# PlanNoa/video_super_resolution

Hardware: NVIDIA B200
Metric: sr_frames_per_s_4x_1080p_out (higher is better)
Workload: dtype bf16

## Files before the change

video_super_resolution_b200/csrc/fused_down.cuh:

```cuda
#pragma once
#include "igemm.cuh"

namespace vsr {

constexpr int kFusedEpiWarps = 16;
constexpr int kFusedWdWarp = 2 + kFusedEpiWarps;
constexpr int kFusedBWarp = kFusedWdWarp + 1;
constexpr int kFusedThreads = 32 * (kFusedBWarp + 1);
constexpr int kFusedMaxStages = 16;
constexpr int kWdGroupBytes = 128 * 128 * 2;
constexpr int kWdRingBytes = 2 * kWdGroupBytes;
constexpr int kWtChunkBytes = 32 * 32 * 2;
constexpr int kHBytes = 128 * 128 * 2;
constexpr int kXchgBytes = 3 * 4 * 16 * 8 * 4;

struct alignas(64) FusedDownParams {
  CUtensorMap hr_maps[kMaxSources];
  CUtensorMap h0_map;
  CUtensorMap wt_map;
  CUtensorMap wd_map;
  int32_t nsrc;
  int32_t num_stages;
  int32_t tiles_x, tiles_y, batch;
  int32_t lr_h, lr_w;
  const float* tran_bias;
  const float* down_bias;
  float* part;
  void* lr_out;
};

__device__ __forceinline__ void tmem_ld8(uint32_t taddr, uint32_t (&v)[8]) {
  asm volatile("tcgen05.ld.sync.aligned.32x32b.x8.b32 {%0, %1, %2, %3, %4, %5, %6, %7}, [%8];"
               : "=r"(v[0]), "=r"(v[1]), "=r"(v[2]), "=r"(v[3]), "=r"(v[4]), "=r"(v[5]), "=r"(v[6]), "=r"(v[7])
               : "r"(taddr)
               : "memory");
}

template <bool HAS_TRAN>
inline size_t fused_down_smem_bytes(int nsrc, int num_stages) {
  size_t wt = HAS_TRAN ? ((size_t)nsrc * kWtChunkBytes + 1023) / 1024 * 1024 : 0;
  size_t stage = HAS_TRAN ? 16384 : 2 * 16384;
  return 1024 + kWdRingBytes + wt + (HAS_TRAN ? kHBytes : 0) + (size_t)num_stages * stage + 1024 + kXchgBytes;
}

template <bool HAS_TRAN>
__global__ void __launch_bounds__(kFusedThreads, 1)
fused_down_kernel(const __grid_constant__ FusedDownParams p) {
  constexpr int kStageBytes = HAS_TRAN ? 16384 : 2 * 16384;
  constexpr int kTmemCols = HAS_TRAN ? 512 : 256;
  constexpr uint32_t kDB = HAS_TRAN ? 256 : 0;

  extern __shared__ uint8_t smem_raw[];
  uint8_t* smem = smem_raw + ((1024u - (smem_u32(smem_raw) & 1023u)) & 1023u);
  uint8_t* s_wd = smem;
  uint8_t* s_wt = s_wd + kWdRingBytes;
  const int wt_region = HAS_TRAN ? ((p.nsrc * kWtChunkBytes + 1023) / 1024 * 1024) : 0;
  uint8_t* s_h = s_wt + wt_region;
  uint8_t* s_a = s_h + (HAS_TRAN ? kHBytes : 0);
  uint8_t* tail = s_a + p.num_stages * kStageBytes;
  uint64_t* full_bar = reinterpret_cast<uint64_t*>(tail);
  uint64_t* empty_bar = full_bar + kFusedMaxStages;
  uint64_t* w_full = empty_bar + kFusedMaxStages;
  uint64_t* wd_full = w_full + 1;
  uint64_t* wd_empty = wd_full + 2;
  uint64_t* da_full = wd_empty + 2;
  uint64_t* da_empty = da_full + 2;
  uint64_t* h_full = da_empty + 2;
  uint64_t* h_empty = h_full + 1;
  uint64_t* db_full = h_empty + 1;
  uint64_t* db_empty = db_full + 2;
  uint32_t* tmem_ptr = reinterpret_cast<uint32_t*>(db_empty + 2);
  float* s_bias = reinterpret_cast<float*>(tail + 512);
  float* s_down = s_bias + 36;
  float4* s_x = reinterpret_cast<float4*>(tail + 1024);

  const int cta = blockIdx.x, ncta = gridDim.x;
  const int warp = threadIdx.x >> 5;
  const int lane = threadIdx.x & 31;
  const int total_tiles = p.tiles_x * p.tiles_y * p.batch;

  if (threadIdx.x == 0) {
    for (int s = 0; s < p.num_stages; ++s) {
      mbar_init(&full_bar[s], 1);
      mbar_init(&empty_bar[s], 1);
    }
    mbar_init(w_full, 1);
    for (int s = 0; s < 2; ++s) {
      mbar_init(&wd_full[s], 1);
      mbar_init(&wd_empty[s], 1);
      mbar_init(&da_full[s], 1);
      mbar_init(&da_empty[s], kFusedEpiWarps);
      mbar_init(&db_full[s], 1);
      mbar_init(&db_empty[s], kFusedEpiWarps);
    }
    mbar_init(h_full, kFusedEpiWarps);
    mbar_init(h_empty, 1);
    fence_barrier_init();
  }
  if (warp == 1) tmem_alloc<kTmemCols>(tmem_ptr);
  if (HAS_TRAN)
    for (int i = threadIdx.x; i < 33; i += kFusedThreads) s_bias[i] = p.tran_bias[i];
  for (int i = threadIdx.x; i < 33; i += kFusedThreads) s_down[i] = p.down_bias[i];
  tc_fence_before();
  __syncthreads();
  tc_fence_after();
  const uint32_t tmem_base = *tmem_ptr;

  auto tile_coord = [&](int tile, int& x0, int& y0, int& b) {
    x0 = (tile % p.tiles_x) * 16;
    int r = tile / p.tiles_x;
    y0 = (r % p.tiles_y) * 8;
    b = r / p.tiles_y;
  };

  if (warp == 0) {
    {
      if (HAS_TRAN && elect_one()) {
        mbar_expect_tx(w_full, (uint32_t)(p.nsrc * kWtChunkBytes));
        for (int j = 0; j < p.nsrc; ++j) tma_load_2d(s_wt + j * kWtChunkBytes, &p.wt_map, w_full, j * 32, 0);
      }
      __syncwarp();
      int s = 0;
      uint32_t phase = 0;
      for (int tile = cta; tile < total_tiles; tile += ncta) {
        int x0, y0, b;
        tile_coord(tile, x0, y0, b);
        for (int half = 0; half < 2; ++half) {
          if (HAS_TRAN) {
            for (int sp = half * 8; sp < half * 8 + 8; sp += 2) {
              for (int j = 0; j < p.nsrc; ++j) {
                mbar_wait(&empty_bar[s], phase ^ 1);
                if (elect_one()) {
                  mbar_expect_tx(&full_bar[s], kStageBytes);
                  tma_load_4d(s_a + s * kStageBytes, &p.hr_maps[j], &full_bar[s], 0, x0, y0, b * 8 + (sp >> 1));
                }
                __syncwarp();
                if (++s == p.num_stages) { s = 0; phase ^= 1; }
              }
            }
          } else {
            for (int g = half * 2; g < half * 2 + 2; ++g) {
              mbar_wait(&empty_bar[s], phase ^ 1);
              if (elect_one()) {
                mbar_expect_tx(&full_bar[s], kStageBytes);
                tma_load_4d(s_a + s * kStageBytes, &p.h0_map, &full_bar[s], 0, x0, y0, b * 8 + 2 * g);
                tma_load_4d(s_a + s * kStageBytes + 16384, &p.h0_map, &full_bar[s], 0, x0, y0, b * 8 + 2 * g + 1);
              }
              __syncwarp();
              if (++s == p.num_stages) { s = 0; phase ^= 1; }
            }
          }
        }
      }
    }
  } else if (warp == 1 || (HAS_TRAN && warp == kFusedBWarp)) {
    {
    constexpr uint32_t idesc_a = make_idesc(32);
    constexpr uint32_t idesc_b = make_idesc(128);
    if (HAS_TRAN && warp == 1) mbar_wait(w_full, 0);
    tc_fence_after();
    int s = 0;
    uint32_t phase = 0;
    uint32_t n_a[2] = {0, 0}, n_b[2] = {0, 0}, n_h = 0, n_wd = 0;
    int tb = 0;
    const uint64_t dA = make_smem_desc<128>(smem_u32(s_a));
    const uint64_t dWt = make_smem_desc<64>(smem_u32(s_wt));
    const uint64_t dH = make_smem_desc<128>(smem_u32(s_h));
    const uint64_t dWd = make_smem_desc<128>(smem_u32(s_wd));

    auto issue_a = [&](int g) {
      const int buf = g & 1;
      mbar_wait(&da_empty[buf], (n_a[buf] & 1) ^ 1);
      tc_fence_after();
      for (int pair = 0; pair < 2; ++pair)
        for (int j = 0; j < p.nsrc; ++j) {
          mbar_wait(&full_bar[s], phase);
          tc_fence_after();
          const uint64_t a0 = dA + (uint64_t)((s * kStageBytes) >> 4);
          const uint64_t b0 = dWt + (uint64_t)((j * kWtChunkBytes) >> 4);
          const uint32_t d0 = tmem_base + (uint32_t)(buf * 128 + pair * 64);
          if (elect_one()) {
            const uint32_t acc = (uint32_t)(j != 0);
            umma_bf16(d0, a0, b0, idesc_a, acc);
            umma_bf16(d0, a0 + 2, b0 + 2, idesc_a, 1u);
            umma_bf16(d0 + 32, a0 + 4, b0, idesc_a, acc);
            umma_bf16(d0 + 32, a0 + 6, b0 + 2, idesc_a, 1u);
            umma_commit(&empty_bar[s]);
            if (pair == 1 && j == p.nsrc - 1) umma_commit(&da_full[buf]);
          }
          __syncwarp();
          if (++s == p.num_stages) { s = 0; phase ^= 1; }
        }
      ++n_a[buf];
    };
    auto issue_b = [&](int g) {
      uint64_t a0;
      if (HAS_TRAN) {
        mbar_wait(h_full, n_h & 1);
        a0 = dH;
      } else {
        mbar_wait(&full_bar[s], phase);
        a0 = dA + (uint64_t)((s * kStageBytes) >> 4);
      }
      if (g == 0) mbar_wait(&db_empty[tb], (n_b[tb] & 1) ^ 1);
      const int wslot = (int)(n_wd & 1);
      mbar_wait(&wd_full[wslot], (n_wd >> 1) & 1);
      tc_fence_after();
      const uint32_t d = tmem_base + kDB + (uint32_t)(tb * 128);
      const uint64_t b0 = dWd + (uint64_t)((wslot * kWdGroupBytes) >> 4);
      if (elect_one()) {
#pragma unroll
        for (int kc = 0; kc < 2; ++kc)
#pragma unroll
          for (int k = 0; k < 4; ++k)
            umma_bf16(d, a0 + (uint64_t)(kc * 1024 + k * 2), b0 + (uint64_t)(kc * 1024 + k * 2), idesc_b,
                      (uint32_t)((g | kc | k) != 0));
        umma_commit(&wd_empty[wslot]);
        if (HAS_TRAN) umma_commit(h_empty);
        else umma_commit(&empty_bar[s]);
        if (g == 3) umma_commit(&db_full[tb]);
      }
      __syncwarp();
      ++n_wd;
      if (HAS_TRAN) ++n_h;
      else if (++s == p.num_stages) { s = 0; phase ^= 1; }
      if (g == 3) { ++n_b[tb]; tb ^= 1; }
    };

    for (int tile = cta; tile < total_tiles; tile += ncta) {
      if (HAS_TRAN) {
        if (warp == 1) {
          for (int g = 0; g < 4; ++g) issue_a(g);
        } else {
          for (int g = 0; g < 4; ++g) issue_b(g);
        }
      } else {
        for (int g = 0; g < 4; ++g) issue_b(g);
      }
    }
    }
  } else if (warp == kFusedWdWarp) {
    uint32_t n_wd = 0;
    for (int tile = cta; tile < total_tiles; tile += ncta)
      for (int g = 0; g < 4; ++g) {
        const int slot = n_wd & 1;
        mbar_wait(&wd_empty[slot], ((n_wd >> 1) & 1) ^ 1);
        if (elect_one()) {
          mbar_expect_tx(&wd_full[slot], kWdGroupBytes);
          tma_load_2d(s_wd + slot * kWdGroupBytes, &p.wd_map, &wd_full[slot], (2 * g) * 64, 0);
          tma_load_2d(s_wd + slot * kWdGroupBytes + 16384, &p.wd_map, &wd_full[slot], (2 * g + 1) * 64, 0);
        }
        __syncwarp();
        ++n_wd;
      }
  } else if (warp >= 2 && warp < 2 + kFusedEpiWarps) {
    const int q = warp & 3;
    const int sub = (warp - 2) >> 2;
    const int row = q * 32 + lane;
    const uint32_t lane_base = tmem_base + ((uint32_t)(q * 32) << 16);
    uint32_t m_a[2] = {0, 0}, m_b[2] = {0, 0}, m_h = 0;
    int tb = 0;
    const PreluCfg pc = make_prelu(HAS_TRAN ? s_bias[32] : 1.0f, 1);
    for (int tile = cta; tile < total_tiles; tile += ncta) {
      int x0, y0, b;
      tile_coord(tile, x0, y0, b);
      const int Yb = y0 + (row >> 4), Xb = x0 + (row & 15);
      const bool in_tensor = (Yb <= p.lr_h) && (Xb <= p.lr_w);
      if (HAS_TRAN) {
#pragma unroll 1
        for (int g = 0; g < 4; ++g) {
          const int buf = g & 1;
          mbar_wait_poll(&da_full[buf], m_a[buf] & 1);
          tc_fence_after();
          uint32_t o[16];
          uint32_t v[32];
          tmem_ld32(lane_base + (uint32_t)(buf * 128 + sub * 32), v);
          tmem_ld_wait();
          tc_fence_before();
          mbar_arrive_warp(&da_empty[buf]);
          const int s16 = g * 4 + sub, ry = s16 >> 2, rx = s16 & 3;
          const bool ring = (Yb == 0 && ry < 2) || (Yb == p.lr_h && ry >= 2) || (Xb == 0 && rx < 2) ||
                            (Xb == p.lr_w && rx >= 2);
          convert32(v, s_bias, pc, o);
          if (__builtin_expect(!(in_tensor && !ring), 0)) zero16(o);
          ++m_a[buf];
          mbar_wait(h_empty, (m_h & 1) ^ 1);
          uint8_t* hrow = s_h + (sub >> 1) * 16384 + (row >> 3) * 1024 + (row & 7) * 128;
#pragma unroll
          for (int j = 0; j < 4; ++j) {
            const int piece = (sub & 1) * 4 + j;
            *reinterpret_cast<uint4*>(hrow + ((piece ^ (row & 7)) << 4)) =
                make_uint4(o[4 * j], o[4 * j + 1], o[4 * j + 2], o[4 * j + 3]);
          }
          fence_async_smem();
          mbar_arrive_warp(h_full);
          ++m_h;
        }
      }
      mbar_wait_poll(&db_full[tb], m_b[tb] & 1);
      tc_fence_after();
      uint32_t v[4][8];
#pragma unroll
      for (int t = 0; t < 4; ++t) tmem_ld8(lane_base + kDB + (uint32_t)(tb * 128 + t * 32 + sub * 8), v[t]);
      tmem_ld_wait();
      tc_fence_before();
      mbar_arrive_warp(&db_empty[tb]);
      const int xl = lane & 15, half = lane >> 4;
      float comb[2][8];
#pragma unroll
      for (int dy = 0; dy < 2; ++dy)
#pragma unroll
        for (int k = 0; k < 8; ++k) {
          const float right = __uint_as_float(v[dy * 2 + 1][k]);
          const float from_right = __shfl_down_sync(0xffffffffu, right, 1);
          comb[dy][k] = __uint_as_float(v[dy * 2][k]) + (xl < 15 ? from_right : 0.0f);
        }
      float below[8];
#pragma unroll
      for (int k = 0; k < 8; ++k) below[k] = __shfl_down_sync(0xffffffffu, comb[1][k], 16);
      if (half == 0 && q > 0) {
        float4* x = s_x + (((q - 1) * 4 + sub) * 16 + xl) * 2;
        x[0] = make_float4(comb[1][0], comb[1][1], comb[1][2], comb[1][3]);
        x[1] = make_float4(comb[1][4], comb[1][5], comb[1][6], comb[1][7]);
      }
      asm volatile("bar.sync 1, %0;" ::"n"(32 * kFusedEpiWarps) : "memory");
      if (half == 1 && q < 3) {
        const float4* x = s_x + ((q * 4 + sub) * 16 + xl) * 2;
        const float4 x0v = x[0], x1v = x[1];
        below[0] = x0v.x; below[1] = x0v.y; below[2] = x0v.z; below[3] = x0v.w;
        below[4] = x1v.x; below[5] = x1v.y; below[6] = x1v.z; below[7] = x1v.w;
      }
      asm volatile("bar.sync 1, %0;" ::"n"(32 * kFusedEpiWarps) : "memory");
      const int rr = 2 * q + half;
      if (rr < 7 && xl < 15 && in_tensor && Yb < p.lr_h && Xb < p.lr_w) {
        const float slope = s_down[32];
        float r[8];
#pragma unroll
        for (int k = 0; k < 8; ++k) r[k] = prelu(comb[0][k] + below[k] + s_down[sub * 8 + k], slope, 1);
        uint4* dst = reinterpret_cast<uint4*>(reinterpret_cast<uint8_t*>(p.lr_out) +
                                               ((((int64_t)b * p.lr_h + Yb) * p.lr_w + Xb) * 64 + sub * 16));
        *dst = make_uint4(pack_bf16(r[0], r[1]), pack_bf16(r[2], r[3]), pack_bf16(r[4], r[5]), pack_bf16(r[6], r[7]));
      }
#pragma unroll
      for (int dy = 0; dy < 2; ++dy) {
        const int Y = Yb - dy;
        if (in_tensor && Y >= 0 && Y < p.lr_h) {
          const bool boundary = (((rr - dy) & 7) == 7) || (xl == 15);
          if (Xb < p.lr_w && boundary) {
            float4* dst = reinterpret_cast<float4*>(p.part + ((((int64_t)b * p.lr_h + Y) * p.lr_w + Xb) * 4 + 2 * dy) * 32 + sub * 8);
            dst[0] = make_float4(comb[dy][0], comb[dy][1], comb[dy][2], comb[dy][3]);
            dst[1] = make_float4(comb[dy][4], comb[dy][5], comb[dy][6], comb[dy][7]);
          }
          if (xl == 0 && Xb > 0) {
            float4* dst = reinterpret_cast<float4*>(p.part + ((((int64_t)b * p.lr_h + Y) * p.lr_w + Xb - 1) * 4 + 2 * dy + 1) * 32 + sub * 8);
            dst[0] = make_float4(__uint_as_float(v[dy * 2 + 1][0]), __uint_as_float(v[dy * 2 + 1][1]),
                                 __uint_as_float(v[dy * 2 + 1][2]), __uint_as_float(v[dy * 2 + 1][3]));
            dst[1] = make_float4(__uint_as_float(v[dy * 2 + 1][4]), __uint_as_float(v[dy * 2 + 1][5]),
                                 __uint_as_float(v[dy * 2 + 1][6]), __uint_as_float(v[dy * 2 + 1][7]));
          }
        }
      }
      ++m_b[tb];
      tb ^= 1;
    }
  }

  tc_fence_before();
  __syncthreads();
  if (warp == 1) {
    tc_fence_after();
    tmem_dealloc<kTmemCols>(tmem_base);
  }
}

constexpr int kFinalizePeriod = 8;
__global__ void __launch_bounds__(256)
finalize_lr_kernel(const float4* __restrict__ part, const float* __restrict__ bias, uint4* __restrict__ out, int B, int h,
                   int w) {
  constexpr int period = kFinalizePeriod;
  const float slope = __ldg(bias + 32);
  const int R = h / period, Cc = w / 16;
  const int64_t nA = (int64_t)B * R * w, nB = (int64_t)B * (h - R) * Cc;
  const int64_t n8 = (nA + nB) * 4;
  for (int64_t i = (int64_t)blockIdx.x * blockDim.x + threadIdx.x; i < n8; i += (int64_t)gridDim.x * blockDim.x) {
    const int c8 = (int)(i & 3);
    int64_t it = i >> 2;
    int b, Y, X;
    if (it < nA) {
      X = (int)(it % w);
      const int64_t r = it / w;
      Y = (int)(r % R) * period + period - 1;
      b = (int)(r / R);
    } else {
      it -= nA;
      X = (int)(it % Cc) * 16 + 15;
      const int64_t r = it / Cc;
      const int yy = (int)(r % (h - R));
      Y = yy + yy / (period - 1);
      b = (int)(r / (h - R));
    }
    const bool last_col = (X & 15) == 15;
    const int64_t px = ((int64_t)b * h + Y) * w + X;
    const float4* base = part + px * 32 + c8 * 2;
    float4 a0 = base[0], a1 = base[1];
    const float4 b0 = base[16], b1 = base[17];
    a0 = make_float4(a0.x + b0.x, a0.y + b0.y, a0.z + b0.z, a0.w + b0.w);
    a1 = make_float4(a1.x + b1.x, a1.y + b1.y, a1.z + b1.z, a1.w + b1.w);
    if (last_col) {
      const float4 c0 = base[8], c1 = base[9], d0 = base[24], d1 = base[25];
      a0 = make_float4(a0.x + (c0.x + d0.x), a0.y + (c0.y + d0.y), a0.z + (c0.z + d0.z), a0.w + (c0.w + d0.w));
      a1 = make_float4(a1.x + (c1.x + d1.x), a1.y + (c1.y + d1.y), a1.z + (c1.z + d1.z), a1.w + (c1.w + d1.w));
    }
    float r[8] = {a0.x, a0.y, a0.z, a0.w, a1.x, a1.y, a1.z, a1.w};
#pragma unroll
    for (int k = 0; k < 8; ++k) r[k] = prelu(r[k] + __ldg(bias + c8 * 8 + k), slope, 1);
    out[px * 4 + c8] = make_uint4(pack_bf16(r[0], r[1]), pack_bf16(r[2], r[3]), pack_bf16(r[4], r[5]), pack_bf16(r[6], r[7]));
  }
}

}
```

video_super_resolution_b200/csrc/srfbn.cu:

```cuda
#include "fused_down.cuh"

#include <string.h>

#include <new>
#include <vector>

namespace vsr {
namespace {

constexpr int kNF = 32;
constexpr int kGroups = 6;
constexpr int kMaxMaps = 64;

typedef CUresult (*EncodeTiledFn)(CUtensorMap*, CUtensorMapDataType, cuuint32_t, void*, const cuuint64_t*,
                                  const cuuint64_t*, const cuuint32_t*, const cuuint32_t*, CUtensorMapInterleave,
                                  CUtensorMapSwizzle, CUtensorMapL2promotion, CUtensorMapFloatOOBfill);

EncodeTiledFn encode_fn() {
  static EncodeTiledFn fn = nullptr;
  if (!fn) {
    void* p = nullptr;
    cudaDriverEntryPointQueryResult q;
    if (cudaGetDriverEntryPoint("cuTensorMapEncodeTiled", &p, cudaEnableDefault, &q) == cudaSuccess &&
        q == cudaDriverEntryPointSuccess)
      fn = reinterpret_cast<EncodeTiledFn>(p);
  }
  return fn;
}

int make_act_map(CUtensorMap* m, const void* base, int64_t C, int64_t W, int64_t H, int64_t B, int ck, int tw, int th) {
  EncodeTiledFn enc = encode_fn();
  if (!enc) return VSR_ERR_STATE;
  cuuint64_t dims[4] = {(cuuint64_t)C, (cuuint64_t)W, (cuuint64_t)H, (cuuint64_t)B};
  cuuint64_t strides[3] = {(cuuint64_t)C * 2, (cuuint64_t)C * 2 * W, (cuuint64_t)C * 2 * W * H};
  cuuint32_t box[4] = {(cuuint32_t)ck, (cuuint32_t)tw, (cuuint32_t)th, 1};
  cuuint32_t es[4] = {1, 1, 1, 1};
  CUresult r = enc(m, CU_TENSOR_MAP_DATA_TYPE_BFLOAT16, 4, const_cast<void*>(base), dims, strides, box, es,
                   CU_TENSOR_MAP_INTERLEAVE_NONE, ck == 32 ? CU_TENSOR_MAP_SWIZZLE_64B : CU_TENSOR_MAP_SWIZZLE_128B,
                   CU_TENSOR_MAP_L2_PROMOTION_L2_128B, CU_TENSOR_MAP_FLOAT_OOB_FILL_NONE);
  return r == CUDA_SUCCESS ? VSR_OK : VSR_ERR_CUDA_BASE + 999;
}

int make_w_map(CUtensorMap* m, const void* base, int64_t K, int64_t N, int ck, int bn) {
  EncodeTiledFn enc = encode_fn();
  if (!enc) return VSR_ERR_STATE;
  cuuint64_t dims[2] = {(cuuint64_t)K, (cuuint64_t)N};
  cuuint64_t strides[1] = {(cuuint64_t)K * 2};
  cuuint32_t box[2] = {(cuuint32_t)ck, (cuuint32_t)bn};
  cuuint32_t es[2] = {1, 1};
  CUresult r = enc(m, CU_TENSOR_MAP_DATA_TYPE_BFLOAT16, 2, const_cast<void*>(base), dims, strides, box, es,
                   CU_TENSOR_MAP_INTERLEAVE_NONE, ck == 32 ? CU_TENSOR_MAP_SWIZZLE_64B : CU_TENSOR_MAP_SWIZZLE_128B,
                   CU_TENSOR_MAP_L2_PROMOTION_L2_256B, CU_TENSOR_MAP_FLOAT_OOB_FILL_NONE);
  return r == CUDA_SUCCESS ? VSR_OK : VSR_ERR_CUDA_BASE + 999;
}

enum Variant : int { V_PW32 = 0, V_PW128, V_DECONV, V_CONVOUT, V_FUSED_TRAN, V_FUSED_PLAIN, V_FINALIZE, V_DECONV2, V_DOWN2, V_COUNT };

static_assert(VSR_SRFBN_KERNEL_CLASSES == 10, "header constant");
enum KClass : int { KC_IM2COL = 0, KC_CONV_IN, KC_PW_LR, KC_PW_HR, KC_DECONV, KC_DOWNCONV, KC_CONV_OUT, KC_FC, KC_FUSED_DOWN, KC_FINALIZE, KC_COUNT };

struct Layer {
  int variant;
  IgemmParams p;
  FusedDownParams f;
  float* fin_acc;
  const float* fin_bias;
  void* fin_out;
  int64_t fin_n8;
  int fin_w, fin_h, fin_b;
  int grid;
  size_t smem;
  int kclass;
  double flops;
  double bytes;
};

template <int MODE, int CK, int BN>
int launch_variant(const Layer& L, cudaStream_t st) {
  static PerDeviceOnce once;
  int dev;
  if (once.needed(&dev)) {
    cudaError_t e = cudaFuncSetAttribute(igemm_kernel<MODE, CK, BN>, cudaFuncAttributeMaxDynamicSharedMemorySize,
                                         227 * 1024);
    if (e != cudaSuccess) return cuda_status(e);
    once.mark(dev);
  }
  igemm_kernel<MODE, CK, BN><<<L.grid, igemm_threads(MODE), L.smem, st>>>(L.p);
  return after_launch();
}

template <bool HAS_TRAN>
int launch_fused(const Layer& L, cudaStream_t st) {
  static PerDeviceOnce once;
  int dev;
  if (once.needed(&dev)) {
    cudaError_t e = cudaFuncSetAttribute(fused_down_kernel<HAS_TRAN>, cudaFuncAttributeMaxDynamicSharedMemorySize,
                                         227 * 1024);
    if (e != cudaSuccess) return cuda_status(e);
    once.mark(dev);
  }
  fused_down_kernel<HAS_TRAN><<<L.grid, kFusedThreads, L.smem, st>>>(L.f);
  return after_launch();
}

int launch_layer(const Layer& L, cudaStream_t st) {
  switch (L.variant) {
    case V_FUSED_TRAN: return launch_fused<true>(L, st);
    case V_FUSED_PLAIN: return launch_fused<false>(L, st);
    case V_FINALIZE: {
      const int R = L.fin_h / kFinalizePeriod;
      const int64_t items = ((int64_t)L.fin_b * R * L.fin_w + (int64_t)L.fin_b * (L.fin_h - R) * (L.fin_w / 16)) * 4;
      if (items == 0) return VSR_OK;
      int64_t blocks = ceil_div64(items, 256);
      if (blocks > kNumSMs * 16) blocks = kNumSMs * 16;
      finalize_lr_kernel<<<(int)blocks, 256, 0, st>>>(reinterpret_cast<const float4*>(L.fin_acc), L.fin_bias,
                                                      reinterpret_cast<uint4*>(L.fin_out), L.fin_b, L.fin_h, L.fin_w);
      return after_launch();
    }
    case V_PW32: return launch_variant<EPI_ROWS, 32, 32>(L, st);
    case V_PW128: return launch_variant<EPI_ROWS, 32, 128>(L, st);
    case V_DECONV: return launch_variant<EPI_DECONV, 32, 256>(L, st);
    case V_CONVOUT: return launch_variant<EPI_CONV_OUT, 32, 32>(L, st);
    case V_DECONV2: return launch_variant<EPI_DECONV2, 32, 128>(L, st);
    case V_DOWN2: return launch_variant<EPI_DOWN2, 64, 96>(L, st);
    default: return VSR_ERR_INVALID_ARG;
  }
}

size_t variant_smem(int variant, int chunks, size_t ring) {
  switch (variant) {
    case V_PW32: return igemm_smem_bytes<32, 32>(chunks, ring);
    case V_PW128: return igemm_smem_bytes<32, 128>(chunks, ring);
    case V_DECONV2: return igemm_smem_bytes<32, 128>(chunks, ring, kDeconv2StageBytes);
    case V_DECONV: return igemm_smem_bytes<32, 256>(chunks, ring, kDeconvStageBytes);
    case V_DOWN2: return igemm_smem_bytes<64, 96>(chunks, ring);
    default: return igemm_smem_bytes<32, 32>(chunks, ring, kConvOutStageBytes);
  }
}

void finish_layer(Layer& L, int ctas_per_sm) {
  IgemmParams& p = L.p;
  if (p.cps < 1) p.cps = 1;
  if (p.stage_bytes == 0) {
    constexpr int kA = a_stage_bytes<32>();
    p.stage_bytes = p.cps * kA;
    for (int i = 0; i < p.num_chunks; ++i) {
      p.chunks[i].a_off = (i % p.cps) * kA;
      p.chunks[i].tx = kA;
    }
  }
  L.smem = variant_smem(L.variant, p.num_chunks, (size_t)p.num_stages * p.stage_bytes);
  int64_t total = (int64_t)p.n_tiles * p.tiles_x * p.tiles_y * p.batch;
  int64_t g = (int64_t)kNumSMs * ctas_per_sm;
  if (g > total) g = total;
  g -= g % p.n_tiles;
  if (g < p.n_tiles) g = p.n_tiles;
  L.grid = (int)g;
}

// ... 218 lines not shown
  const double lrpx = (double)B * h * w;
  L.kclass = KC_DOWNCONV;
  L.flops = lrpx * 73728.0;
  L.bytes = lrpx * 64.0 * 5.0;
  return VSR_OK;
}

int build_fused_down(Layer& L, const void* const* hr, int nsrc, int B, int h, int w, const void* wt_dev,
                     const float* tran_bias_dev, const void* wd_dev, const float* down_bias_dev, float* part,
                     void* lr_out) {
  memset(&L, 0, sizeof(L));
  const bool tran = nsrc > 1;
  L.variant = tran ? V_FUSED_TRAN : V_FUSED_PLAIN;
  FusedDownParams& f = L.f;
  if (nsrc < 1 || nsrc > kMaxSources) return VSR_ERR_UNSUPPORTED;
  int rc;
  if (tran) {
    for (int j = 0; j < nsrc; ++j) {
      rc = make_act_map(&f.hr_maps[j], hr[j], 64, w + 1, h + 1, 8 * B, 64, 16, 8);
      if (rc) return rc;
    }
    rc = make_w_map(&f.wt_map, wt_dev, 32 * nsrc, 32, 32, 32);
    if (rc) return rc;
  } else {
    rc = make_act_map(&f.h0_map, hr[0], 64, w + 1, h + 1, 8 * B, 64, 16, 8);
    if (rc) return rc;
  }
  rc = make_w_map(&f.wd_map, wd_dev, 512, 128, 64, 128);
  if (rc) return rc;
  f.nsrc = nsrc;
  f.num_stages = tran ? 7 : 5;
  f.tiles_x = ceil_div(w + 1, 16);
  f.tiles_y = ceil_div(h + 1, 8);
  f.batch = B;
  f.lr_h = h;
  f.lr_w = w;
  f.tran_bias = tran_bias_dev;
  f.down_bias = down_bias_dev;
  f.part = part;
  f.lr_out = lr_out;
  while (f.num_stages > 2 && (tran ? fused_down_smem_bytes<true>(nsrc, f.num_stages)
                                   : fused_down_smem_bytes<false>(nsrc, f.num_stages)) > 227 * 1024)
    --f.num_stages;
  L.smem = tran ? fused_down_smem_bytes<true>(nsrc, f.num_stages) : fused_down_smem_bytes<false>(nsrc, f.num_stages);
  int64_t total = (int64_t)f.tiles_x * f.tiles_y * B;
  L.grid = (int)(total < kNumSMs ? total : kNumSMs);
  const double lrpx = (double)B * h * w;
  L.kclass = KC_FUSED_DOWN;
  L.flops = lrpx * 131072.0 + (tran ? lrpx * 16.0 * 2.0 * 32.0 * nsrc * 32.0 : 0.0);
  L.bytes = lrpx * 64.0 * (16.0 * nsrc) + lrpx * 64.0;
  return VSR_OK;
}

int build_finalize(Layer& L, float* acc, const float* bias_dev, void* out, int64_t pixels, int h, int w) {
  memset(&L, 0, sizeof(L));
  L.variant = V_FINALIZE;
  L.fin_acc = acc;
  L.fin_bias = bias_dev;
  L.fin_out = out;
  L.fin_n8 = pixels * 4;
  L.fin_w = w;
  L.fin_h = h;
  L.fin_b = (int)(pixels / ((int64_t)h * w));
  L.kclass = KC_FINALIZE;
  L.flops = 0;
  L.bytes = 0;
  return VSR_OK;
}

int build_conv_out(Layer& L, const void* xhr, int B, int h, int w, int scale, const void* w_dev,
                   const float* bias_dev, float* out) {
  memset(&L, 0, sizeof(L));
  L.variant = V_CONVOUT;
  IgemmParams& p = L.p;
  const int H = scale * h, W = scale * w;
  p.inv_scale = 1.0f / (float)scale;
  int rc = make_act_map(&p.a_maps[0], xhr, kNF, W, H, B, 32, 16, 8);
  if (rc) return rc;
  rc = make_w_map(&p.b_map, w_dev, kNF, 32, 32, 32);
  if (rc) return rc;
  p.chunks[0].map = 0;
  p.chunks[0].dx = p.chunks[0].dy = 0;
  p.chunks[0].c0 = 0;
  p.num_chunks = 1;
  p.num_stages = 3;
  p.n_tiles = 1;
  p.tile_w = 14;
  p.tile_h = 6;
  p.org_x = -1;
  p.org_y = -1;
  p.tiles_x = ceil_div(W, 14);
  p.tiles_y = ceil_div(H, 6);
  p.batch = B;
  p.bias = bias_dev;
  p.bias_n = 16;
  p.act = 0;
  p.out = out;
  p.out_h = H;
  p.out_w = W;
  p.lr_h = h;
  p.lr_w = w;
  finish_layer(L, 3);
  const double hrpx = (double)B * H * W;
  L.kclass = KC_CONV_OUT;
  L.flops = hrpx * 2.0 * 288 * 3;
  L.bytes = hrpx * (64.0 + 12.0) + hrpx / (scale * scale) * 12.0;
// ... 201 lines not shown
  std::vector<Layer> refresh_layers;
  int refresh_first, refresh_conv_out_layer;
  bool premix_valid;
  std::vector<cudaEvent_t> events;
  bool profile;
};

static void layout_weights(vsr_srfbn_plan* pl) {
  size_t off = 0;
  auto put = [&](int id, int N, int K, int bias_floats) {
    pl->we[id].N = N;
    pl->we[id].K = K;
    pl->we[id].w_off = off;
    off = align_up(off + (size_t)N * K * 2, 256);
    pl->we[id].b_off = off;
    off = align_up(off + (size_t)bias_floats * 4, 256);
  };
  put(W_CONV_IN, 128, 32, 129);
  put(W_FEAT_IN, 32, 128, 33);
  put(W_COMPRESS_IN, 32, 64, 33);
  for (int i = 0; i < 5; ++i) put(W_UPTRAN0 + i, 32, 32 * (i + 2), 33);
  const bool x2 = pl->cfg.upscale == 2;
  for (int i = 0; i < 6; ++i) put(W_UP0 + i, x2 ? 128 : 512, x2 ? 288 : 128, 33);
  for (int i = 0; i < 5; ++i) put(W_DOWNTRAN0 + i, 32, 32 * (i + 2), 33);
  for (int i = 0; i < 6; ++i) put(W_DOWN0 + i, x2 ? 96 : 128, x2 ? 384 : 512, 33);
  put(W_COMPRESS_OUT, 32, 192, 33);
  put(W_OUT, x2 ? 128 : 512, x2 ? 288 : 128, 33);
  put(W_CONV_OUT, 32, 32, 16 + 7);
  pl->fc_off = off;
  off = align_up(off + (size_t)(32 * pl->cfg.num_maps + 65) * 4, 256);
  pl->misc_off = off;
  off = align_up(off + 16, 256);
  pl->weight_bytes = off;
}

static void layout_workspace(vsr_srfbn_plan* pl) {
  const vsr_srfbn_config& c = pl->cfg;
  const size_t P = (size_t)pl->chunk_maps * c.h * c.w;
  const size_t Rb = (size_t)pl->chunk_maps * (c.h + 1) * (c.w + 1) * 16;
  size_t off = 0;
  auto put = [&](size_t bytes) {
    size_t o = off;
    off = align_up(off + bytes, 1024);
    return o;
  };
  pl->o_a0 = put(P * 64);
  pl->o_c128 = put(P * 256);
  pl->o_xfeat = put(P * 64);
  pl->o_hidden = put(P * 64);
  for (int i = 0; i < 7; ++i) pl->o_lr[i] = put(P * 64);
  pl->o_u = put(P * 64);
  const size_t s2 = (size_t)c.upscale * c.upscale;
  const bool x2 = c.upscale == 2;
  for (int i = 0; i < 6; ++i) pl->o_hr[i] = put(x2 ? P * s2 * 64 : Rb * 64);
  pl->o_hb = put(P * s2 * 64);
  pl->o_ht = put(x2 ? P * s2 * 64 : 0);
  pl->o_acc = put(x2 ? 0 : P * 512);
  pl->o_premix = put((size_t)c.num_maps * c.h * c.w * s2 * 3 * 4);
  pl->ws_bytes = off;
}

extern "C" int vsr_srfbn_plan_create(const vsr_srfbn_config* cfg, vsr_srfbn_plan** out_plan) {
  if (!cfg || !out_plan) return VSR_ERR_INVALID_ARG;
  *out_plan = nullptr;
  if (cfg->num_maps < 1 || cfg->h < 1 || cfg->w < 1 || cfg->num_steps < 1) return VSR_ERR_INVALID_ARG;
  if (cfg->num_groups != kGroups || cfg->num_features != kNF || (cfg->upscale != 4 && cfg->upscale != 2) ||
      cfg->num_maps > kMaxMaps)
    return VSR_ERR_UNSUPPORTED;
  vsr_srfbn_plan* pl = new (std::nothrow) vsr_srfbn_plan();
  if (!pl) return VSR_ERR_INVALID_ARG;
  pl->cfg = *cfg;
  pl->bound = false;
  pl->dev_w = nullptr;
  pl->ws = nullptr;
  pl->conv_out_layer = -1;
  pl->refresh_first = -1;
  pl->refresh_conv_out_layer = -1;
  pl->premix_valid = false;
  pl->profile = false;
  pl->chunk_maps = cfg->num_maps;
  pl->ws_cap = 0;
  layout_weights(pl);
  layout_workspace(pl);
  *out_plan = pl;
  return VSR_OK;
}

extern "C" int vsr_srfbn_plan_set_workspace_cap(vsr_srfbn_plan* pl, size_t cap_bytes) {
  if (!pl) return VSR_ERR_INVALID_ARG;
  if (pl->bound) return VSR_ERR_STATE;
  pl->ws_cap = cap_bytes;
  const int M = pl->cfg.num_maps;
  for (int mc = M; mc >= 1; --mc) {
    if (M % mc) continue;
    pl->chunk_maps = mc;
    layout_workspace(pl);
    if (cap_bytes == 0 || pl->ws_bytes <= cap_bytes) return VSR_OK;
  }
  return VSR_ERR_WORKSPACE;
}

extern "C" int vsr_srfbn_chunk_maps(const vsr_srfbn_plan* pl) { return pl ? pl->chunk_maps : 0; }

extern "C" void vsr_srfbn_plan_destroy(vsr_srfbn_plan* plan) {
  if (!plan) return;
  for (cudaEvent_t e : plan->events) cudaEventDestroy(e);
  delete plan;
// ... 90 lines not shown
  const vsr_srfbn_config& c = pl->cfg;
  const int h = c.h, w = c.w;
  const int64_t P = (int64_t)M * h * w;
  uint8_t* ws = pl->ws;
  auto Wp = [&](int id) { return (const void*)(pl->dev_w + pl->we[id].w_off); };
  auto Bp = [&](int id) { return reinterpret_cast<const float*>(pl->dev_w + pl->we[id].b_off); };
  int rc;
  Layer L;
#define PUSH(expr)        \
  do {                    \
    rc = (expr);          \
    if (rc) return rc;    \
    layers.push_back(L);  \
  } while (0)

  {
    Src s{ws + pl->o_a0, 32, 0, 32};
    PUSH(build_pointwise(L, &s, 1, P, Wp(W_CONV_IN), Bp(W_CONV_IN), 128, 1, ws + pl->o_c128, 256, 0, 0, h, w));
  }
  {
    Src s{ws + pl->o_c128, 128, 0, 128};
    PUSH(build_pointwise(L, &s, 1, P, Wp(W_FEAT_IN), Bp(W_FEAT_IN), 32, 1, ws + pl->o_xfeat, 64, 0, 0, h, w));
  }
  for (int step = 0; step < c.num_steps; ++step) {
    {
      Src s[2] = {{ws + pl->o_xfeat, 32, 0, 32}, {ws + (step == 0 ? pl->o_xfeat : pl->o_hidden), 32, 0, 32}};
      PUSH(build_pointwise(L, s, 2, P, Wp(W_COMPRESS_IN), Bp(W_COMPRESS_IN), 32, 1, ws + pl->o_lr[0], 64, 0, 0, h, w));
    }
    for (int i = 0; i < kGroups; ++i) {
      const void* up_in = ws + pl->o_lr[0];
      if (i > 0) {
        Src s[6];
        for (int j = 0; j <= i; ++j) s[j] = Src{ws + pl->o_lr[j], 32, 0, 32};
        PUSH(build_pointwise(L, s, i + 1, P, Wp(W_UPTRAN0 + i - 1), Bp(W_UPTRAN0 + i - 1), 32, 1, ws + pl->o_u, 64, 0,
                             0, h, w));
        up_in = ws + pl->o_u;
      }
      if (c.upscale == 2) {
        PUSH(build_deconv2(L, up_in, M, h, w, Wp(W_UP0 + i), Bp(W_UP0 + i), ws + pl->o_hr[i]));
        const void* down_in = ws + pl->o_hr[0];
        if (i > 0) {
          Src s[6];
          for (int j = 0; j <= i; ++j) s[j] = Src{ws + pl->o_hr[j], 32, 0, 32};
          rc = build_pointwise(L, s, i + 1, P * 4, Wp(W_DOWNTRAN0 + i - 1), Bp(W_DOWNTRAN0 + i - 1), 32, 1,
                               ws + pl->o_ht, 64, 0, 0, h, w);
          if (rc) return rc;
          L.kclass = KC_PW_HR;
          layers.push_back(L);
          down_in = ws + pl->o_ht;
        }
        PUSH(build_downconv2(L, down_in, M, h, w, Wp(W_DOWN0 + i), Bp(W_DOWN0 + i), ws + pl->o_lr[i + 1]));
        continue;
      }
      {
        Layer D, F;
        rc = build_deconv(D, up_in, M, h, w, Wp(W_UP0 + i), Bp(W_UP0 + i), ws + pl->o_hr[i], 0);
        if (rc) return rc;
        const void* hrs[6];
        for (int j = 0; j <= i; ++j) hrs[j] = ws + pl->o_hr[j];
        rc = build_fused_down(F, hrs, i + 1, M, h, w, i > 0 ? Wp(W_DOWNTRAN0 + i - 1) : nullptr,
                              i > 0 ? Bp(W_DOWNTRAN0 + i - 1) : nullptr, Wp(W_DOWN0 + i), Bp(W_DOWN0 + i),
                              reinterpret_cast<float*>(ws + pl->o_acc), ws + pl->o_lr[i + 1]);
        if (rc) return rc;
        layers.push_back(D);
        layers.push_back(F);
        PUSH(build_finalize(L, reinterpret_cast<float*>(ws + pl->o_acc), Bp(W_DOWN0 + i), ws + pl->o_lr[i + 1], P, h, w));
      }
    }
    {
      Src s[6];
      for (int j = 0; j < 6; ++j) s[j] = Src{ws + pl->o_lr[j + 1], 32, 0, 32};
      PUSH(build_pointwise(L, s, 6, P, Wp(W_COMPRESS_OUT), Bp(W_COMPRESS_OUT), 32, 1, ws + pl->o_hidden, 64, 0, 0, h,
                           w));
    }
  }
  if (c.upscale == 2) PUSH(build_deconv2(L, ws + pl->o_hidden, M, h, w, Wp(W_OUT), Bp(W_OUT), ws + pl->o_hb));
  else PUSH(build_deconv(L, ws + pl->o_hidden, M, h, w, Wp(W_OUT), Bp(W_OUT), ws + pl->o_hb, 1));
  PUSH(build_conv_out(L, ws + pl->o_hb, M, h, w, c.upscale, Wp(W_CONV_OUT), Bp(W_CONV_OUT),
                      reinterpret_cast<float*>(ws + pl->o_premix)));
  conv_out_layer = (int)layers.size() - 1;
#undef PUSH
  return VSR_OK;
}

extern "C" int vsr_srfbn_prepare_refresh(vsr_srfbn_plan* pl, int first_map) {
  if (!pl) return VSR_ERR_INVALID_ARG;
  if (!pl->bound) return VSR_ERR_STATE;
  if (first_map < 1 || first_map >= pl->cfg.num_maps) return VSR_ERR_INVALID_ARG;
  if (pl->chunk_maps != pl->cfg.num_maps) return VSR_ERR_UNSUPPORTED;
  if (pl->refresh_first == first_map) return VSR_OK;
  pl->refresh_first = -1;
  const int rc = build_layer_list(pl, pl->cfg.num_maps - first_map, pl->refresh_layers, pl->refresh_conv_out_layer);
  if (rc) return rc;
  pl->refresh_first = first_map;
  return VSR_OK;
}

extern "C" int vsr_srfbn_forward(vsr_srfbn_plan* pl, const float* x, float* y, vsr_stream_t stream) {
  return vsr_srfbn_forward_u8(pl, x, y, nullptr, stream);
}

static int sweep_maps(vsr_srfbn_plan* pl, std::vector<Layer>& layers, int conv_out_layer, const float* x, int m0, int Mc,
                      cudaStream_t st, size_t* ev) {
  const vsr_srfbn_config& c = pl->cfg;
  const int64_t P = (int64_t)Mc * c.h * c.w;
  auto mark = [&]() {
    if (ev && pl->profile && *ev < pl->events.size()) cudaEventRecord(pl->events[(*ev)++], st);
// ... 266 lines not shown
```

Baseline: 11.10.

## Fuse up-projection deconv into the fused down kernel for later groups

For back-projection groups with four or more sources, the deconvolution that produces the newest HR feature map now runs inside the fused down kernel. It is computed from a tile of LR input via an extra UMMA into TMEM, converted in the epilogue, and fed straight to the transition GEMM from shared memory. This removes a separate kernel launch and the HR round trip through global memory; the last group skips the HR store entirely and its buffer is no longer allocated. In exchange, the down path loses TMEM double-buffering and the weight ring gets a single slot, and extra barriers serialize the epilogue warps, which may reduce overlap.

```diff
diff --git a/video_super_resolution_b200/csrc/fused_down.cuh b/video_super_resolution_b200/csrc/fused_down.cuh
--- a/video_super_resolution_b200/csrc/fused_down.cuh
+++ b/video_super_resolution_b200/csrc/fused_down.cuh
@@ -13,6 +13,9 @@
 constexpr int kWtChunkBytes = 32 * 32 * 2;
 constexpr int kHBytes = 128 * 128 * 2;
 constexpr int kXchgBytes = 3 * 4 * 16 * 8 * 4;
+constexpr int kLRBox = 16 * 9 * 64;
+constexpr int kLRBytes = 2 * kLRBox;
+constexpr int kWuTapBytes = 128 * 32 * 2;
 
 struct alignas(64) FusedDownParams {
   CUtensorMap hr_maps[kMaxSources];
@@ -27,6 +30,10 @@
   const float* down_bias;
   float* part;
   void* lr_out;
+  CUtensorMap up_map;
+  CUtensorMap wu_map;
+  const float* up_bias;
+  int32_t hr_store;
 };
 
 __device__ __forceinline__ void tmem_ld8(uint32_t taddr, uint32_t (&v)[8]) {
@@ -43,12 +50,18 @@
   return 1024 + kWdRingBytes + wt + (HAS_TRAN ? kHBytes : 0) + (size_t)num_stages * stage + 1024 + kXchgBytes;
 }
 
-template <bool HAS_TRAN>
-__global__ void __launch_bounds__(kFusedThreads, 1)
-fused_down_kernel(const __grid_constant__ FusedDownParams p) {
+inline size_t fused_updown_smem_bytes(int nsrc, int num_stages) {
+  return fused_down_smem_bytes<true>(nsrc, num_stages) + kLRBytes;
+}
+
+template <bool HAS_TRAN, bool MERGED>
+__device__ __forceinline__ void fused_down_body(const FusedDownParams& p) {
+  static_assert(HAS_TRAN || !MERGED, "the merged kernel needs phase A");
   constexpr int kStageBytes = HAS_TRAN ? 16384 : 2 * 16384;
   constexpr int kTmemCols = HAS_TRAN ? 512 : 256;
-  constexpr uint32_t kDB = HAS_TRAN ? 256 : 0;
+  constexpr uint32_t kDB = MERGED ? 384 : HAS_TRAN ? 256 : 0;
+  constexpr int kDBToggle = MERGED ? 0 : 1;
+  constexpr uint32_t kTU = 256;
 
   extern __shared__ uint8_t smem_raw[];
   uint8_t* smem = smem_raw + ((1024u - (smem_u32(smem_raw) & 1023u)) & 1023u);
@@ -56,7 +69,8 @@
   uint8_t* s_wt = s_wd + kWdRingBytes;
   const int wt_region = HAS_TRAN ? ((p.nsrc * kWtChunkBytes + 1023) / 1024 * 1024) : 0;
   uint8_t* s_h = s_wt + wt_region;
-  uint8_t* s_a = s_h + (HAS_TRAN ? kHBytes : 0);
+  uint8_t* s_lr = s_h + (HAS_TRAN ? kHBytes : 0);
+  uint8_t* s_a = s_lr + (MERGED ? kLRBytes : 0);
   uint8_t* tail = s_a + p.num_stages * kStageBytes;
   uint64_t* full_bar = reinterpret_cast<uint64_t*>(tail);
   uint64_t* empty_bar = full_bar + kFusedMaxStages;
@@ -70,8 +84,14 @@
   uint64_t* db_full = h_empty + 1;
   uint64_t* db_empty = db_full + 2;
   uint32_t* tmem_ptr = reinterpret_cast<uint32_t*>(db_empty + 2);
+  uint64_t* tu_full = db_empty + 3;
+  uint64_t* tu_empty = tu_full + 1;
+  uint64_t* u_full = tu_empty + 1;
+  uint64_t* lr_full = u_full + 1;
+  uint64_t* lr_empty = lr_full + 1;
   float* s_bias = reinterpret_cast<float*>(tail + 512);
   float* s_down = s_bias + 36;
+  float* s_ubias = s_down + 36;
   float4* s_x = reinterpret_cast<float4*>(tail + 1024);
 
   const int cta = blockIdx.x, ncta = gridDim.x;
@@ -95,11 +115,20 @@
     }
     mbar_init(h_full, kFusedEpiWarps);
     mbar_init(h_empty, 1);
+    if (MERGED) {
+      mbar_init(tu_full, 1);
+      mbar_init(tu_empty, kFusedEpiWarps);
+      mbar_init(u_full, 1);
+      mbar_init(lr_full, 1);
+      mbar_init(lr_empty, 1);
+    }
     fence_barrier_init();
   }
   if (warp == 1) tmem_alloc<kTmemCols>(tmem_ptr);
   if (HAS_TRAN)
     for (int i = threadIdx.x; i < 33; i += kFusedThreads) s_bias[i] = p.tran_bias[i];
+  if (MERGED)
+    for (int i = threadIdx.x; i < 33; i += kFusedThreads) s_ubias[i] = p.up_bias[i];
   for (int i = threadIdx.x; i < 33; i += kFusedThreads) s_down[i] = p.down_bias[i];
   tc_fence_before();
   __syncthreads();
@@ -128,7 +157,7 @@
         for (int half = 0; half < 2; ++half) {
           if (HAS_TRAN) {
             for (int sp = half * 8; sp < half * 8 + 8; sp += 2) {
-              for (int j = 0; j < p.nsrc; ++j) {
+              for (int j = 0; j < p.nsrc - (MERGED ? 1 : 0); ++j) {
                 mbar_wait(&empty_bar[s], phase ^ 1);
                 if (elect_one()) {
                   mbar_expect_tx(&full_bar[s], kStageBytes);
@@ -167,13 +196,38 @@
     const uint64_t dWt = make_smem_desc<64>(smem_u32(s_wt));
     const uint64_t dH = make_smem_desc<128>(smem_u32(s_h));
     const uint64_t dWd = make_smem_desc<128>(smem_u32(s_wd));
+    uint32_t n_tu = 0, n_lr = 0, n_u = 0;
+
+    auto issue_u = [&](int g) {
+      constexpr uint32_t idesc_u = make_idesc(128);
+      const uint64_t dLR = make_smem_desc<64>(smem_u32(s_lr));
+      const uint64_t dWu = make_smem_desc<64>(smem_u32(s_wd));
+      if (g == 0) mbar_wait(lr_full, n_lr & 1);
+      mbar_wait(tu_empty, (n_tu & 1) ^ 1);
+      mbar_wait(&wd_full[0], n_tu & 1);
+      tc_fence_after();
+      if (elect_one()) {
+#pragma unroll
+        for (int t = 0; t < 4; ++t)
+#pragma unroll
+          for (int k = 0; k < 2; ++k)
+            umma_bf16(tmem_base + kTU, dLR + (uint64_t)(((t & 1) * kLRBox + (t >> 1) * 1024) >> 4) + 2 * k,
+                      dWu + (uint64_t)((t * kWuTapBytes) >> 4) + 2 * k, idesc_u, (uint32_t)((t | k) != 0));
+        umma_commit(&wd_empty[0]);
+        umma_commit(tu_full);
+        if (g == 3) umma_commit(lr_empty);
+      }
+      __syncwarp();
+      ++n_tu;
+      if (g == 3) ++n_lr;
+    };
 
     auto issue_a = [&](int g) {
       const int buf = g & 1;
       mbar_wait(&da_empty[buf], (n_a[buf] & 1) ^ 1);
       tc_fence_after();
       for (int pair = 0; pair < 2; ++pair)
-        for (int j = 0; j < p.nsrc; ++j) {
+        for (int j = 0; j < p.nsrc - (MERGED ? 1 : 0); ++j) {
           mbar_wait(&full_bar[s], phase);
           tc_fence_after();
           const uint64_t a0 = dA + (uint64_t)((s * kStageBytes) >> 4);
@@ -186,11 +240,29 @@
             umma_bf16(d0 + 32, a0 + 4, b0, idesc_a, acc);
             umma_bf16(d0 + 32, a0 + 6, b0 + 2, idesc_a, 1u);
             umma_commit(&empty_bar[s]);
-            if (pair == 1 && j == p.nsrc - 1) umma_commit(&da_full[buf]);
+            if (!MERGED && pair == 1 && j == p.nsrc - 1) umma_commit(&da_full[buf]);
           }
           __syncwarp();
           if (++s == p.num_stages) { s = 0; phase ^= 1; }
         }
+      if (MERGED) {
+        mbar_wait(u_full, n_u & 1);
+        tc_fence_after();
+        const uint64_t b0 = dWt + (uint64_t)(((p.nsrc - 1) * kWtChunkBytes) >> 4);
+        if (elect_one()) {
+          for (int pair = 0; pair < 2; ++pair) {
+            const uint64_t a0 = dH + (uint64_t)((pair * 16384) >> 4);
+            const uint32_t d0 = tmem_base + (uint32_t)(buf * 128 + pair * 64);
+            umma_bf16(d0, a0, b0, idesc_a, 1u);
+            umma_bf16(d0, a0 + 2, b0 + 2, idesc_a, 1u);
+            umma_bf16(d0 + 32, a0 + 4, b0, idesc_a, 1u);
+            umma_bf16(d0 + 32, a0 + 6, b0 + 2, idesc_a, 1u);
+          }
+          umma_commit(&da_full[buf]);
+        }
+        __syncwarp();
+        ++n_u;
+      }
       ++n_a[buf];
     };
     auto issue_b = [&](int g) {
@@ -203,8 +275,8 @@
         a0 = dA + (uint64_t)((s * kStageBytes) >> 4);
       }
       if (g == 0) mbar_wait(&db_empty[tb], (n_b[tb] & 1) ^ 1);
-      const int wslot = (int)(n_wd & 1);
-      mbar_wait(&wd_full[wslot], (n_wd >> 1) & 1);
+      const int wslot = MERGED ? 1 : (int)(n_wd & 1);
+      mbar_wait(&wd_full[wslot], MERGED ? (n_wd & 1) : ((n_wd >> 1) & 1));
       tc_fence_after();
       const uint32_t d = tmem_base + kDB + (uint32_t)(tb * 128);
       const uint64_t b0 = dWd + (uint64_t)((wslot * kWdGroupBytes) >> 4);
@@ -224,13 +296,16 @@
       ++n_wd;
       if (HAS_TRAN) ++n_h;
       else if (++s == p.num_stages) { s = 0; phase ^= 1; }
-      if (g == 3) { ++n_b[tb]; tb ^= 1; }
+      if (g == 3) { ++n_b[tb]; tb ^= kDBToggle; }
     };
 
     for (int tile = cta; tile < total_tiles; tile += ncta) {
       if (HAS_TRAN) {
         if (warp == 1) {
-          for (int g = 0; g < 4; ++g) issue_a(g);
+          for (int g = 0; g < 4; ++g) {
+            if (MERGED) issue_u(g);
+            issue_a(g);
+          }
         } else {
           for (int g = 0; g < 4; ++g) issue_b(g);
         }
@@ -239,6 +314,43 @@
       }
     }
     }
+  } else if (MERGED && warp == kFusedWdWarp) {
+    uint32_t n_wu = 0, n_wdm = 0, n_lrl = 0;
+    auto load_u = [&](int tile, int g) {
+      if (g == 0) {
+        int x0, y0, b;
+        tile_coord(tile, x0, y0, b);
+        mbar_wait(lr_empty, (n_lrl & 1) ^ 1);
+        if (elect_one()) {
+          mbar_expect_tx(lr_full, (uint32_t)kLRBytes);
+          tma_load_4d(s_lr, &p.up_map, lr_full, 0, x0 - 1, y0 - 1, b);
+          tma_load_4d(s_lr + kLRBox, &p.up_map, lr_full, 0, x0, y0 - 1, b);
+        }
+        __syncwarp();
+        ++n_lrl;
+      }
+      mbar_wait(&wd_empty[0], (n_wu & 1) ^ 1);
+      if (elect_one()) {
+        mbar_expect_tx(&wd_full[0], kWdGroupBytes);
+        for (int t = 0; t < 4; ++t) tma_load_2d(s_wd + t * kWuTapBytes, &p.wu_map, &wd_full[0], t * 32, g * 128);
+      }
+      __syncwarp();
+      ++n_wu;
+    };
+    if (cta < total_tiles) load_u(cta, 0);
+    for (int tile = cta; tile < total_tiles; tile += ncta)
+      for (int g = 0; g < 4; ++g) {
+        if (g < 3) load_u(tile, g + 1);
+        else if (tile + ncta < total_tiles) load_u(tile + ncta, 0);
+        mbar_wait(&wd_empty[1], (n_wdm & 1) ^ 1);
+        if (elect_one()) {
+          mbar_expect_tx(&wd_full[1], kWdGroupBytes);
+          tma_load_2d(s_wd + kWdGroupBytes, &p.wd_map, &wd_full[1], (2 * g) * 64, 0);
+          tma_load_2d(s_wd + kWdGroupBytes + 16384, &p.wd_map, &wd_full[1], (2 * g + 1) * 64, 0);
+        }
+        __syncwarp();
+        ++n_wdm;
+      }
   } else if (warp == kFusedWdWarp) {
     uint32_t n_wd = 0;
     for (int tile = cta; tile < total_tiles; tile += ncta)
@@ -261,6 +373,7 @@
     uint32_t m_a[2] = {0, 0}, m_b[2] = {0, 0}, m_h = 0;
     int tb = 0;
     const PreluCfg pc = make_prelu(HAS_TRAN ? s_bias[32] : 1.0f, 1);
+    uint32_t m_u = 0;
     for (int tile = cta; tile < total_tiles; tile += ncta) {
       int x0, y0, b;
       tile_coord(tile, x0, y0, b);
@@ -270,6 +383,41 @@
 #pragma unroll 1
         for (int g = 0; g < 4; ++g) {
           const int buf = g & 1;
+          if (MERGED) {
+            mbar_wait_poll(tu_full, m_u & 1);
+            tc_fence_after();
+            uint32_t v[32];
+            tmem_ld32(lane_base + kTU + (uint32_t)(sub * 32), v);
+            tmem_ld_wait();
+            tc_fence_before();
+            mbar_arrive_warp(tu_empty);
+            ++m_u;
+            const int s16 = g * 4 + sub, ry = s16 >> 2, rx = s16 & 3;
+            const int Yt = 4 * Yb + ry - 2, Xt = 4 * Xb + rx - 2;
+            const bool inside = (Yt >= 0) && (Yt < 4 * p.lr_h) && (Xt >= 0) && (Xt < 4 * p.lr_w);
+            uint32_t o[16];
+            const PreluCfg pcu = make_prelu(s_ubias[32], 1);
+            convert32(v, s_ubias, pcu, o);
+            if (__builtin_expect(!inside, 0)) zero16(o);
+            mbar_wait(h_empty, (m_h & 1) ^ 1);
+            uint8_t* urow = s_h + (sub >> 1) * 16384 + row * 128;
+#pragma unroll
+            for (int j = 0; j < 4; ++j) {
+              const int piece = (sub & 1) * 4 + j;
+              *reinterpret_cast<uint4*>(urow + ((piece ^ (row & 7)) << 4)) =
+                  make_uint4(o[4 * j], o[4 * j + 1], o[4 * j + 2], o[4 * j + 3]);
+            }
+            fence_async_smem();
+            asm volatile("bar.sync 1, %0;" ::"n"(32 * kFusedEpiWarps) : "memory");
+            if (threadIdx.x == 64) {
+              if (p.hr_store) {
+                tma_store_4d(&p.hr_maps[p.nsrc - 1], s_h, 0, x0, y0, b * 8 + 2 * g);
+                tma_store_4d(&p.hr_maps[p.nsrc - 1], s_h + 16384, 0, x0, y0, b * 8 + 2 * g + 1);
+                tma_store_commit();
+              }
+              mbar_arrive(u_full);
+            }
+          }
           mbar_wait_poll(&da_full[buf], m_a[buf] & 1);
           tc_fence_after();
           uint32_t o[16];
@@ -284,7 +432,14 @@
           convert32(v, s_bias, pc, o);
           if (__builtin_expect(!(in_tensor && !ring), 0)) zero16(o);
           ++m_a[buf];
-          mbar_wait(h_empty, (m_h & 1) ^ 1);
+          if (MERGED) {
+            if (p.hr_store) {
+              if (threadIdx.x == 64) tma_store_wait_read();
+              asm volatile("bar.sync 1, %0;" ::"n"(32 * kFusedEpiWarps) : "memory");
+            }
+          } else {
+            mbar_wait(h_empty, (m_h & 1) ^ 1);
+          }
           uint8_t* hrow = s_h + (sub >> 1) * 16384 + (row >> 3) * 1024 + (row & 7) * 128;
 #pragma unroll
           for (int j = 0; j < 4; ++j) {
@@ -361,8 +516,9 @@
         }
       }
       ++m_b[tb];
-      tb ^= 1;
-    }
+      tb ^= kDBToggle;
+    }
+    if (MERGED && threadIdx.x == 64) asm volatile("cp.async.bulk.wait_group 0;" ::: "memory");
   }
 
   tc_fence_before();
@@ -371,6 +527,17 @@
     tc_fence_after();
     tmem_dealloc<kTmemCols>(tmem_base);
   }
+}
+
+template <bool HAS_TRAN>
+__global__ void __launch_bounds__(kFusedThreads, 1)
+fused_down_kernel(const __grid_constant__ FusedDownParams p) {
+  fused_down_body<HAS_TRAN, false>(p);
+}
+
+__global__ void __launch_bounds__(kFusedThreads, 1)
+fused_updown_kernel(const __grid_constant__ FusedDownParams p) {
+  fused_down_body<true, true>(p);
 }
 
 constexpr int kFinalizePeriod = 8;
diff --git a/video_super_resolution_b200/csrc/srfbn.cu b/video_super_resolution_b200/csrc/srfbn.cu
--- a/video_super_resolution_b200/csrc/srfbn.cu
+++ b/video_super_resolution_b200/csrc/srfbn.cu
@@ -54,7 +54,7 @@
   return r == CUDA_SUCCESS ? VSR_OK : VSR_ERR_CUDA_BASE + 999;
 }
 
-enum Variant : int { V_PW32 = 0, V_PW128, V_DECONV, V_CONVOUT, V_FUSED_TRAN, V_FUSED_PLAIN, V_FINALIZE, V_DECONV2, V_DOWN2, V_COUNT };
+enum Variant : int { V_PW32 = 0, V_PW128, V_DECONV, V_CONVOUT, V_FUSED_TRAN, V_FUSED_PLAIN, V_FINALIZE, V_DECONV2, V_DOWN2, V_FUSED_UPDOWN, V_COUNT };
 
 static_assert(VSR_SRFBN_KERNEL_CLASSES == 10, "header constant");
 enum KClass : int { KC_IM2COL = 0, KC_CONV_IN, KC_PW_LR, KC_PW_HR, KC_DECONV, KC_DOWNCONV, KC_CONV_OUT, KC_FC, KC_FUSED_DOWN, KC_FINALIZE, KC_COUNT };
@@ -103,8 +103,21 @@
   return after_launch();
 }
 
+int launch_fused_updown(const Layer& L, cudaStream_t st) {
+  static PerDeviceOnce once;
+  int dev;
+  if (once.needed(&dev)) {
+    cudaError_t e = cudaFuncSetAttribute(fused_updown_kernel, cudaFuncAttributeMaxDynamicSharedMemorySize, 227 * 1024);
+    if (e != cudaSuccess) return cuda_status(e);
+    once.mark(dev);
+  }
+  fused_updown_kernel<<<L.grid, kFusedThreads, L.smem, st>>>(L.f);
+  return after_launch();
+}
+
 int launch_layer(const Layer& L, cudaStream_t st) {
   switch (L.variant) {
+    case V_FUSED_UPDOWN: return launch_fused_updown(L, st);
     case V_FUSED_TRAN: return launch_fused<true>(L, st);
     case V_FUSED_PLAIN: return launch_fused<false>(L, st);
     case V_FINALIZE: {
@@ -429,6 +442,52 @@
   return VSR_OK;
 }
 
+inline bool updown_merged(int nsrc) { return nsrc >= 4; }
+
+int build_fused_updown(Layer& L, const void* up_in, const void* const* hr, int nsrc, int store, int B, int h, int w,
+                       const void* wu_dev, const float* up_bias_dev, const void* wt_dev, const float* tran_bias_dev,
+                       const void* wd_dev, const float* down_bias_dev, float* part, void* lr_out) {
+  memset(&L, 0, sizeof(L));
+  L.variant = V_FUSED_UPDOWN;
+  FusedDownParams& f = L.f;
+  if (nsrc < 2 || nsrc > kMaxSources || (store && !hr[nsrc - 1])) return VSR_ERR_UNSUPPORTED;
+  int rc;
+  for (int j = 0; j < nsrc - (store ? 0 : 1); ++j) {
+    rc = make_act_map(&f.hr_maps[j], hr[j], 64, w + 1, h + 1, 8 * B, 64, 16, 8);
+    if (rc) return rc;
+  }
+  rc = make_w_map(&f.wt_map, wt_dev, 32 * nsrc, 32, 32, 32);
+  if (rc) return rc;
+  rc = make_w_map(&f.wd_map, wd_dev, 512, 128, 64, 128);
+  if (rc) return rc;
+  rc = make_act_map(&f.up_map, up_in, kNF, w, h, B, 32, kTW, kTH + 1);
+  if (rc) return rc;
+  rc = make_w_map(&f.wu_map, wu_dev, 4 * kNF, 512, 32, 128);
+  if (rc) return rc;
+  f.nsrc = nsrc;
+  f.tiles_x = ceil_div(w + 1, 16);
+  f.tiles_y = ceil_div(h + 1, 8);
+  f.batch = B;
+  f.lr_h = h;
+  f.lr_w = w;
+  f.tran_bias = tran_bias_dev;
+  f.down_bias = down_bias_dev;
+  f.up_bias = up_bias_dev;
+  f.part = part;
+  f.lr_out = lr_out;
+  f.hr_store = store;
+  const int64_t total = (int64_t)f.tiles_x * f.tiles_y * B;
+  L.grid = (int)(total < kNumSMs ? total : kNumSMs);
+  f.num_stages = 7;
+  while (f.num_stages > 2 && fused_updown_smem_bytes(nsrc, f.num_stages) > 227 * 1024) --f.num_stages;
+  L.smem = fused_updown_smem_bytes(nsrc, f.num_stages);
+  const double lrpx = (double)B * h * w;
+  L.kclass = KC_FUSED_DOWN;
+  L.flops = lrpx * 131072.0 * 2.0 + lrpx * 16.0 * 2.0 * 32.0 * nsrc * 32.0;
+  L.bytes = lrpx * 64.0 + lrpx * 64.0 * 16.0 * (nsrc - 1 + (store ? 1 : 0)) + lrpx * 64.0;
+  return VSR_OK;
+}
+
 int build_finalize(Layer& L, float* acc, const float* bias_dev, void* out, int64_t pixels, int h, int w) {
   memset(&L, 0, sizeof(L));
   L.variant = V_FINALIZE;
@@ -736,7 +795,7 @@
   pl->o_u = put(P * 64);
   const size_t s2 = (size_t)c.upscale * c.upscale;
   const bool x2 = c.upscale == 2;
-  for (int i = 0; i < 6; ++i) pl->o_hr[i] = put(x2 ? P * s2 * 64 : Rb * 64);
+  for (int i = 0; i < 6; ++i) pl->o_hr[i] = put(x2 ? P * s2 * 64 : (i == 5 && updown_merged(6)) ? 0 : Rb * 64);
   pl->o_hb = put(P * s2 * 64);
   pl->o_ht = put(x2 ? P * s2 * 64 : 0);
   pl->o_acc = put(x2 ? 0 : P * 512);
@@ -933,7 +992,16 @@
         PUSH(build_downconv2(L, down_in, M, h, w, Wp(W_DOWN0 + i), Bp(W_DOWN0 + i), ws + pl->o_lr[i + 1]));
         continue;
       }
-      {
+      if (updown_merged(i + 1)) {
+        const void* hrs[6];
+        for (int j = 0; j <= i; ++j) hrs[j] = ws + pl->o_hr[j];
+        const int store = i + 1 < kGroups;
+        if (!store) hrs[i] = nullptr;
+        PUSH(build_fused_updown(L, up_in, hrs, i + 1, store, M, h, w, Wp(W_UP0 + i), Bp(W_UP0 + i),
+                                Wp(W_DOWNTRAN0 + i - 1), Bp(W_DOWNTRAN0 + i - 1), Wp(W_DOWN0 + i), Bp(W_DOWN0 + i),
+                                reinterpret_cast<float*>(ws + pl->o_acc), ws + pl->o_lr[i + 1]));
+        PUSH(build_finalize(L, reinterpret_cast<float*>(ws + pl->o_acc), Bp(W_DOWN0 + i), ws + pl->o_lr[i + 1], P, h, w));
+      } else {
         Layer D, F;
         rc = build_deconv(D, up_in, M, h, w, Wp(W_UP0 + i), Bp(W_UP0 + i), ws + pl->o_hr[i], 0);
         if (rc) return rc;
```

Result: faster. 11.69 (median of 6 runs) (+5.3%).
